# carlosmwh1985/BspAtom

Hardware: AMD Instinct MI355X
Metric: l-channel eigensolves/sec at N_bsp=4096 fp64 (higher is better)
Workload: dtype f64; 1 GPU; Hydrogen Coulomb l=0..127, N_bsp=4096, k=9, KIND_GRID=0 rb=800 (BASELINE configs[3]); `value` = weak scaling: 128 l-channels per GPU, 128 in total; channels_total=128, eigenvector_owner_rank=0, collective_calls=0, launched_by=python

## Files before the change

bspatom_amd/csrc/capi.hip:

```cpp
#include <atomic>
#include <new>
#include "capi_internal.h"

using namespace bsp;

namespace bsp {
static std::atomic<int> g_process_device{-1};
int process_device() { return g_process_device.load(); }
int process_device_check(int device)
{
    const int cur = g_process_device.load();
    if (cur >= 0 && cur != device) {
        fprintf(stderr, "bspatom: this process already works on device %d; use one process per GPU (device %d refused)\n", cur, device);
        return BSP_ERR_UNSUPPORTED;
    }
    return BSP_OK;
}
void process_device_latch(int device) { int expect = -1; g_process_device.compare_exchange_strong(expect, device); }
}

namespace {
struct OptName { const char *name; const char *env; int Options::*field; };
const OptName OPT_TABLE[] = {
    {"sb2st_version", "BSP_SB2ST_VERSION", &Options::sb2st_version},
    {"sb2st_ring", "BSP_SB2ST_RING", &Options::sb2st_ring},
    {"sb2st_margin", "BSP_SB2ST_MARGIN", &Options::sb2st_margin},
    {"sb2st_hyst", "BSP_SB2ST_HYST", &Options::sb2st_hyst},
    {"sb2st_lead", "BSP_SB2ST_LEAD", &Options::sb2st_lead},
    {"sb2st_check", "BSP_SB2ST_CHECK", &Options::sb2st_check},
    {"sb2st_diag", "BSP_SB2ST_DIAG", &Options::sb2st_diag},
    {"sb2st_force_abort", "BSP_SB2ST_FORCE_ABORT", &Options::sb2st_force_abort},
    {"sy2sb_groups", "BSP_SY2SB_GROUPS", &Options::sy2sb_groups},
    {"sy2sb_lookahead", "BSP_SY2SB_LOOKAHEAD", &Options::sy2sb_lookahead},
    {"sy2sb_segs", "BSP_SY2SB_SEGS", &Options::sy2sb_segs},
    {"panel_qr", "BSP_PANEL_QR", &Options::panel_qr},
    {"gemm_diag", "BSP_GEMM_DIAG", &Options::gemm_diag},
    {"bisect", "BSP_BISECT", &Options::bisect},
    {"bisect_ept", "BSP_BISECT_EPT", &Options::bisect_ept},
    {"bisect_tail", "BSP_BISECT_TAIL", &Options::bisect_tail},
    {"bisect_secant", "BSP_BISECT_SECANT", &Options::bisect_secant},
    {"bisect_pair", "BSP_BISECT_PAIR", &Options::bisect_pair},
    {"bisect_queue", "BSP_BISECT_QUEUE", &Options::bisect_queue},
    {"bisect_queue_grid", "BSP_BISECT_QUEUE_GRID", &Options::bisect_queue_grid},
    {"bisect_diag", "BSP_BISECT_DIAG", &Options::bisect_diag},
    {"no_eigvec_prefetch", "BSP_NO_EIGVEC_PREFETCH", &Options::no_eigvec_prefetch},
    {"vec_early", "BSP_VEC_EARLY", &Options::vec_early},
    {"vec_own_cu", "BSP_VEC_OWN_CU", &Options::vec_own_cu},
    {"poison_c", "BSP_POISON_C", &Options::poison_c},
    {"sb2sb_mfma", "BSP_SB2SB_MFMA", &Options::sb2sb_mfma},
    {"ktime", "BSP_KTIME", &Options::ktime},
    {"tsqr_regcap", "BSP_TSQR_REGCAP", &Options::tsqr_regcap},
    {"tsqr_max_m", "BSP_TSQR_MAX_M", &Options::tsqr_max_m},
    {"sb16_rows", "BSP_SB16_ROWS", &Options::sb16_rows},
    {"route", "BSP_ROUTE", &Options::route},
    {"cw_onediv", "BSP_CW_ONEDIV", &Options::cw_onediv},
    {"cw_items4", "BSP_CW_ITEMS4", &Options::cw_items4},
    {"cw_nw", "BSP_CW_NW", &Options::cw_nw},
    {"cw_ldspad", "BSP_CW_LDSPAD", &Options::cw_ldspad},
    {"cw_ipw", "BSP_CW_IPW", &Options::cw_ipw},
    {"cw_band8", "BSP_CW_BAND8", &Options::cw_band8},
    {"cw_split", "BSP_CW_SPLIT", &Options::cw_split},
    {"cw_diag", "BSP_CW_DIAG", &Options::cw_diag},
    {"s_overlap", "BSP_S_OVERLAP", &Options::s_overlap},
    {"cw_streams", "BSP_CW_STREAMS", &Options::cw_streams},
    {"cw_chunk_min", "BSP_CW_CHUNK_MIN", &Options::cw_chunk_min},
    {"sb8_wgs", "BSP_SB8_WGS", &Options::sb8_wgs},
    {"sbr_phased", "BSP_SBR_PHASED", &Options::sbr_phased},
    {"sbr_lag", "BSP_SBR_LAG", &Options::sbr_lag},
    {"fused_probe", "BSP_FUSED_PROBE", &Options::fused_probe},
    {"dipole_stage_mb", "BSP_DIPOLE_STAGE_MB", &Options::dipole_stage_mb},
    {"wf_stage_mb", "BSP_WF_STAGE_MB", &Options::wf_stage_mb},
    {"tdse_stage_mb", "BSP_TDSE_STAGE_MB", &Options::tdse_stage_mb},
    {"tdse_adapt_group", "BSP_TDSE_ADAPT_GROUP", &Options::tdse_adapt_group},
};
}

namespace bsp {
Options &opts()
{
    static Options o = [] {
        Options v;
        for (const OptName &t : OPT_TABLE) {
            const char *e = getenv(t.env);
            if (e) v.*(t.field) = (*e == 0) ? 1 : atoi(e);
        }
        return v;
    }();
    return o;
}

namespace {
struct KRec { int slot; hipEvent_t e0, e1; };
std::vector<KRec> g_krecs;
std::vector<hipEvent_t> g_kpool;
hipEvent_t g_kopen[KS_COUNT];
hipEvent_t kevent()
{
    hipEvent_t e = nullptr;
    if (!g_kpool.empty()) { e = g_kpool.back(); g_kpool.pop_back(); }
    else if (hipEventCreate(&e) != hipSuccess) e = nullptr;
    return e;
}
const char *const KSLOT_NAMES[KS_COUNT] = {"gemm2_kernel<128,128,MODE 1> (rank-128 update, syr2k)", "gemm2_kernel<64,128,MODE 2> (symm Y = A22 W)",
                                          "panel_qr2_kernel / panel_qr_kernel", "sy2sb chain: G, K (split-K gemm_kernel + splitk_reduce), form_T, tsmm64 (W, Z)",
                                          "sb2sb_mfma_kernel (band 64 -> 16)", "sbr_rows_kernel<8> / <16> / sb16st_kernel (one-column chase to tridiagonal)", "bisect3_kernel",
                                          "band_cholesky_kernel + std_form_kernel",
                                          "crawford_item_kernel and its set-up kernels (band route: pencil -> band 15)",
                                          "operator_band_kernel (bands of caller-given g(r), g(r) d/dr)",
                                          "tdse_stage_kernel (one Runge-Kutta stage of bspatom_tdse_propagate)"};
}
void ktime_begin(int slot, hipStream_t st)
{
    hipEvent_t e = kevent();
    g_kopen[slot] = e;
    if (e) (void)hipEventRecord(e, st);
}
void ktime_end(int slot, hipStream_t st)
{
    hipEvent_t e0 = g_kopen[slot], e1 = kevent();
    g_kopen[slot] = nullptr;
    if (!e0 || !e1) return;
    (void)hipEventRecord(e1, st);
    g_krecs.push_back({slot, e0, e1});
}
}

extern "C" int bspatom_kernel_times(double *ms, int32_t *launches, int cap)
{
    if (!ms || !launches || cap < KS_COUNT) return BSP_ERR_ARG;
    BSP_HIP(hipDeviceSynchronize());
    for (int i = 0; i < cap; ++i) { ms[i] = 0.0; launches[i] = 0; }
    for (const auto &r : g_krecs) {
        float t = 0.f;
        if (hipEventElapsedTime(&t, r.e0, r.e1) == hipSuccess) { ms[r.slot] += t; launches[r.slot] += 1; }
        g_kpool.push_back(r.e0); g_kpool.push_back(r.e1);
    }
    g_krecs.clear();
    return KS_COUNT;
}
// ... 469 lines not shown
```

bspatom_amd/csrc/common.h:

```cpp
#pragma once
#include <hip/hip_runtime.h>
#include <cstdint>
#include <cstdio>
#include <cstdlib>

#define BSP_OK 0
#define BSP_ERR_HIP (-1)
#define BSP_ERR_ARG (-2)
#define BSP_ERR_BSPLVB (-3)
#define BSP_ERR_NOGPU (-4)
#define BSP_ERR_UNSUPPORTED (-5)

#define BSP_HIP(x)                                                                          \
    do {                                                                                    \
        hipError_t e_ = (x);                                                                \
        if (e_ != hipSuccess) {                                                             \
            fprintf(stderr, "bspatom: HIP error '%s' at %s:%d\n", hipGetErrorString(e_),    \
                    __FILE__, __LINE__);                                                    \
            return BSP_ERR_HIP;                                                             \
        }                                                                                   \
    } while (0)

typedef double double4_t __attribute__((ext_vector_type(4)));

__host__ __device__ inline size_t ab_stride(int npad) { return (size_t)npad * 128 + 1088; }

namespace bsp {

struct Options {
    int sb2st_version = 0;
    int sb2st_ring = 0;
    int sb2st_margin = 3, sb2st_hyst = 2;
    int sb2st_lead = 0;
    int sb2st_check = 0;
    int sb2st_diag = 0;
    int sb2st_force_abort = 0;
    int sy2sb_groups = 2, sy2sb_lookahead = 1, sy2sb_segs = 0;
    int panel_qr = 3;
    int tsqr_max_m = 2048;
    int tsqr_regcap = 1;
    int gemm_diag = 0;
    int bisect = 3, bisect_ept = 0;
    int bisect_secant = 1;
    int bisect_tail = 1;
    int bisect_pair = 1;
    int bisect_queue = 1;
    int bisect_queue_grid = 0;
    int bisect_diag = 0;
    int no_eigvec_prefetch = 0;
    int vec_early = 1;
    int vec_own_cu = 1;
    int sb2sb_mfma = 1;
    int sb16_rows = 1;
    int poison_c = 0;
    int route = 0;
    int fused_probe = 0;
    int cw_items4 = 1;
    int cw_nw = 1;
    int cw_streams = 2;
    int cw_chunk_min = 1024;
    int s_overlap = 1;
    int cw_diag = 0;
    int cw_split = 0;
    int cw_band8 = 1;
    int sb8_wgs = 0;
    int sbr_phased = 1;
    int sbr_lag = 0;
    int cw_ipw = 0;
    int cw_ldspad = 0;
    int cw_onediv = 0;
    int dipole_stage_mb = 0;
    int wf_stage_mb = 0;
    int tdse_stage_mb = 0;
    int tdse_adapt_group = 0;
    int ktime = 0;
};
Options &opts();

int process_device();
int process_device_check(int device);
void process_device_latch(int device);

enum KSlot { KS_SYR2K = 0, KS_SYMM, KS_PANEL_QR, KS_CHAIN, KS_SB2SB, KS_SB16ST, KS_BISECT, KS_STDFORM, KS_CRAWFORD, KS_OPBAND, KS_TDSE, KS_COUNT };
void ktime_begin(int slot, hipStream_t st);
void ktime_end(int slot, hipStream_t st);
struct KScope {
    int slot; hipStream_t st; bool on;
    KScope(int slot_, hipStream_t st_) : slot(slot_), st(st_), on(opts().ktime != 0) { if (on) ktime_begin(slot, st); }
    ~KScope() { if (on) ktime_end(slot, st); }
};

struct GemmDesc {
    int M, N, K, batch;
    const double *A; long sAm, sAk, bA;
    const double *B; long sBk, sBn, bB;
    double *C; long sCm, sCn, bC;
    double alpha, beta;
    int lower_only;
    int yoff;
    int ksplit;
    int kchunk;
    long bCs;
    int nsb, toff;
    int sbpre[80];
    int sbxy[80];
};
int gemm_f64(const GemmDesc &g, hipStream_t st);
int gemm_splitk_f64(const GemmDesc &g, int splits, double *part, hipStream_t st);
int tsmm64_f64(int m, int batch, const double *A, long lda, long bsA, const double *B, long bsB, double *C, long ldc, long bsC,
               double alpha, double beta, hipStream_t st);
int syr2k_lower_f64(int m, int batch, double *A22, long ld, long bsA, const double *buf, long ldb, long bsBuf, int seg, int nseg,
                    int part, hipStream_t st);
int symm_lower_f64(int m, int batch, const double *A22, long ld, long bsA, const double *W, long ldw, long bsW,
                   double *Y, long ldy, long bsY, hipStream_t st);

int launch_point_table(int nkp, int k, int ka, int nfun, const double *d_rt, const double *d_aind,
                       const double *d_xg, const double *d_wg, const double *d_vpot, double *d_ptab,
                       int *d_left, int *d_status, hipStream_t st);
int launch_assemble_bands(int nfun, int k, int ka, int nkp, int kind_pot, const double *d_bl, int l0,
                          int nl, const double *d_ptab, const int *d_left, double *d_SB, double *d_HB,
                          hipStream_t st);
int launch_dipole_bands(int nfun, int k, int ka, int nkp, const double *d_ptab, const int *d_left, double *d_RB,
                        hipStream_t st);
int launch_band_cholesky(int n, int k, const double *d_SB, double *d_UB, double *d_rdiag, int *d_info,
                         hipStream_t st);
int launch_band_cholesky_range(int n, int k, int jstart, int jstop, const double *d_SB, double *d_UB, double *d_rdiag, int *d_info,
                               hipStream_t st);
int launch_band_cholesky_pair(int n, int k, int jstop, const double *d_SB, double *d_UB, double *d_rdiag, int *d_info, hipStream_t st);
int launch_standard_form(int n, int npad, int k, int nl, const double *d_HB, const double *d_UB,
                         const double *d_rdiag, double *d_Y, double *d_C, hipStream_t st, int full = 0);
struct CrawfordWork {
    double *SBf, *UBf, *rdiagf;
    double *Qel, *LiB;
    double *D, *E, *G;
    int *info;
};
bool crawford_supported(int n, int k);
size_t crawford_work_bytes(int n, int k, int nl);
void crawford_carve(void *base, int n, int k, int nl, CrawfordWork *w);
constexpr int CW_CHUNKS = 4;
int crawford_prepare(int n, int k, const double *d_SB, const CrawfordWork &w, hipStream_t st, hipEvent_t *evc = nullptr);
int crawford_run(int n, int npad, int k, int nl, const double *d_SB, const double *d_HB, const CrawfordWork &w, double *d_AB,
                 hipStream_t st, bool s_prepared = false, hipEvent_t *evc = nullptr, hipStream_t aux0 = nullptr);
long tsqr_scr_doubles(int npad);
long tsqr_cntr_ints(int npad);
int tsqr_panel(int npad, int r0, int c0, int batch, double *d_A, double *buf, double *W, double *scr, int *cntr, hipStream_t st);
struct Sy2sbWork {
    double *tsqr_scr;
    int *tsqr_cntr;
    double *buf2;
    double *tau2;
    double *buf;
    double *W;
// ... 124 lines not shown
```

bspatom_amd/csrc/crawford.hip:

```cpp
#include "common.h"
#include <cstdio>
#include <mutex>

namespace bsp {
namespace {

constexpr int CB = 8;
constexpr int CBB = CB * CB;

template <int CTRL>
__device__ __forceinline__ double cw_dpp(double x)
{
    union { double d; int i[2]; } u, r;
    u.d = x;
    r.i[0] = __builtin_amdgcn_update_dpp(0, u.i[0], CTRL, 0xf, 0xf, true);
    r.i[1] = __builtin_amdgcn_update_dpp(0, u.i[1], CTRL, 0xf, 0xf, true);
    return r.d;
}
__device__ __forceinline__ double cw_rowsum(double x)
{
    x += cw_dpp<0x128>(x);
    x += cw_dpp<0x124>(x);
    x += cw_dpp<0x122>(x);
    x += cw_dpp<0x121>(x);
// ... 146 lines not shown
        for (int r = 0; r < 2; ++r) {
            if (!elim) Em[(4 * r + g) * CB + c8] = O[r];
            Gm[(4 * r + g) * CB + c8] = O[r + 2];
        }
    }
    if (!elim) {
        if (!left) {
            double *E1 = E + (size_t)(p + 1) * CBB;
            E1[g * CB + c8] = x0;
            E1[(4 + g) * CB + c8] = x1;
        }
    } else if (has_x) {
        double4_t T = {0.0, 0.0, 0.0, 0.0};
        T = cw_mfma(q[2], xt[0], T);
        T = cw_mfma(q[3], xt[1], T);
        if (left) {
            double *Ej = E + (size_t)j * CBB;
#pragma unroll
            for (int r = 0; r < 2; ++r) Ej[c8 * CB + 4 * r + g] = T[r + 2];
        }
    }
}

constexpr int QLD = 18;

template <int I, bool ONEDIV>
__device__ __forceinline__ void rq4_step(double (&x)[16], double (&q)[16], double *bc, const int r)
{
    constexpr int LEN = CB + I;
    if (r == I) {
#pragma unroll
        for (int c = 0; c < 16; c += 2) *reinterpret_cast<double2 *>(bc + c) = make_double2(x[c], x[c + 1]);
    }
    asm volatile("" ::: "memory");
    double u[16];
#pragma unroll
    for (int c = 0; c < 16; c += 2) {
        if (c <= LEN) {
            const double2 v = *reinterpret_cast<const double2 *>(bc + c);
            u[c] = v.x; u[c + 1] = v.y;
        }
    }
    asm volatile("" ::: "memory");
    double sg[4] = {0.0, 0.0, 0.0, 0.0};
#pragma unroll
    for (int c = 0; c < LEN; ++c) sg[c & 3] = fma(u[c], u[c], sg[c & 3]);
    const double sig = (sg[0] + sg[1]) + (sg[2] + sg[3]);
    const double alpha = u[LEN];
    const double a2s = fma(alpha, alpha, sig);
    const bool ok = (a2s > 1e-280) && (sig != 0.0);
    const double nrm = sqrt(ok ? a2s : 1.0);
    const double bt = (alpha >= 0.0) ? -nrm : nrm;
    const double amb = alpha - bt;
    const double okf = ok ? 1.0 : 0.0, ambs = ok ? amb : 1.0, bts = ok ? bt : 1.0;
    const double sc = ONEDIV ? 1.0 : (1.0 / ambs) * okf;
    const double t = (ONEDIV ? -1.0 / (bts * ambs) : (bts - alpha) / bts) * okf;
    const double beta = ok ? bt : alpha;
    if (!ONEDIV) {
#pragma unroll
        for (int c = 0; c < LEN; ++c) u[c] *= sc;
    }
    u[LEN] = ONEDIV ? amb : 1.0;
    {
        double ws[4] = {0.0, 0.0, 0.0, 0.0};
#pragma unroll
        for (int c = 0; c <= LEN; ++c) ws[c & 3] = fma(x[c], u[c], ws[c & 3]);
        const double w = (ws[0] + ws[1]) + (ws[2] + ws[3]);
        const double tw = (r <= I) ? -t * w : 0.0;
#pragma unroll
        for (int c = 0; c <= LEN; ++c) x[c] = fma(tw, u[c], x[c]);
    }
    (void)beta;
    {
        double ws[4] = {0.0, 0.0, 0.0, 0.0};
#pragma unroll
        for (int c = 0; c <= LEN; ++c) ws[c & 3] = fma(q[c], u[c], ws[c & 3]);
        const double w = (ws[0] + ws[1]) + (ws[2] + ws[3]);
        const double tw = -t * w;
#pragma unroll
        for (int c = 0; c <= LEN; ++c) q[c] = fma(tw, u[c], q[c]);
    }
}

template <bool ONEDIV>
__device__ __forceinline__ void cw_quad(const int N, const int t, const int jlo, int nch, int jel, const int ipw, const int nlh,
                                        const int qstride, const int nlead, const int chan, const int idx0, const int lane,
                                        double *Qsw, double *Bcw, double *Wsw, const double *__restrict__ Qel, double *Dall, double *Eall,
                                        double *Gall, unsigned long long *diag)
{
    unsigned long long ts0 = 0, tsa = 0, tsb = 0, tsc = 0, tsd = 0, tse = 0;
    if (diag) ts0 = __builtin_amdgcn_s_memtime();
    if (chan >= nlh) {
        if (jlo + nch > nlead) nch = nlead > jlo ? nlead - jlo : 0;
        if (jel >= nlead) jel = 0;
    }
    const int items = nch + (jel > 0 ? 1 : 0);
    if (idx0 >= items) return;
    const size_t chn = (size_t)chan * N * CBB;
    double *D = Dall + chn, *E = Eall + chn, *G = Gall + chn;

#pragma unroll
    for (int s = 0; s < 4; ++s) {
        const int idx = idx0 + s;
        const int kd = s >= ipw ? 0 : (idx < nch ? 1 : ((idx == nch && jel > 0) ? 2 : 0));
        if (kd != 0) {
            const int jx = kd == 1 ? jlo + idx : jel, p = kd == 2 ? jel - 1 : jx - 2 - (t - 2 * jx);
            const double *srcD = D + (size_t)p * CBB + 2 * lane;
            const double *srcE = E + (size_t)((lane < 32 || p < 1) ? p : p - 1) * CBB + 2 * (lane & 31);
            const unsigned ldsD = (unsigned)(size_t)(__attribute__((address_space(3))) void *)(Wsw + s * 4 * CBB);
            asm volatile("s_mov_b32 m0, %2\n\ts_nop 0\n\tglobal_load_lds_dwordx4 %0, off\n\t"
                         "s_mov_b32 m0, %3\n\ts_nop 0\n\tglobal_load_lds_dwordx4 %1, off"
                         :: "v"(srcD), "v"(srcE), "s"(ldsD), "s"(ldsD + 2 * CBB * 8) : "memory", "m0");
        }
    }

    if (idx0 < nch) {
        const int it = lane >> 4, r = lane & 15;
        const int idx = idx0 + it;
        const bool live = idx < nch && it < ipw && r < CB;
        const int j = jlo + (idx < nch ? idx : 0), p = j - 2 - (t - 2 * j);
        double x[16], q[16];
        {
            const double *gp = G + (size_t)p * CBB + (r & 7) * CB, *ep = E + (size_t)(p + 1) * CBB + (r & 7) * CB;
#pragma unroll
            for (int c = 0; c < CB; c += 2) {
                const double2 a = *reinterpret_cast<const double2 *>(gp + c), b = *reinterpret_cast<const double2 *>(ep + c);
                x[c] = live ? a.x : 0.0; x[c + 1] = live ? a.y : 0.0;
                x[CB + c] = live ? b.x : 0.0; x[CB + c + 1] = live ? b.y : 0.0;
            }
        }
#pragma unroll
        for (int c = 0; c < 16; ++c) q[c] = (c == r) ? 1.0 : 0.0;
        double *bc = Bcw + it * 16;
        if (diag) { asm volatile("s_waitcnt vmcnt(0)" ::: "memory"); tsa = __builtin_amdgcn_s_memtime(); }
        rq4_step<7, ONEDIV>(x, q, bc, r);
        rq4_step<6, ONEDIV>(x, q, bc, r);
        rq4_step<5, ONEDIV>(x, q, bc, r);
        rq4_step<4, ONEDIV>(x, q, bc, r);
        rq4_step<3, ONEDIV>(x, q, bc, r);
        rq4_step<2, ONEDIV>(x, q, bc, r);
        rq4_step<1, ONEDIV>(x, q, bc, r);
        rq4_step<0, ONEDIV>(x, q, bc, r);
        if (diag) { asm volatile("s_waitcnt lgkmcnt(0)" ::: "memory"); tsb = __builtin_amdgcn_s_memtime(); }
        if (live) {
            double *ep = E + (size_t)(p + 1) * CBB + r * CB;
#pragma unroll
            for (int c = 0; c < CB; c += 2) *reinterpret_cast<double2 *>(ep + c) = make_double2(x[CB + c], x[CB + c + 1]);
        }
        double *qs = Qsw + it * (16 * QLD) + r * QLD;
#pragma unroll
        for (int c = 0; c < 16; c += 2) *reinterpret_cast<double2 *>(qs + c) = make_double2(q[c], q[c + 1]);
    }
    if (idx0 < nch) asm volatile("s_waitcnt vmcnt(4) lgkmcnt(0)" ::: "memory");
    else asm volatile("s_waitcnt vmcnt(0) lgkmcnt(0)" ::: "memory");
    if (diag) tsc = __builtin_amdgcn_s_memtime();
    int idx0b = idx0;
    size_t chnb = chn;
    asm volatile("" : "+s"(idx0b), "+s"(chnb));
    D = Dall + chnb; E = Eall + chnb; G = Gall + chnb;

    const int g = lane >> 4, c = lane & 15, c8 = c & 7;
    const bool left = c < CB;
    int kind[4], jj[4], pp[4];
    double wv[4][4], sdv[4][2], qe[4], xt[2] = {0.0, 0.0};
#pragma unroll
    for (int s = 0; s < 4; ++s) {
        const int idx = idx0b + s;
        kind[s] = s >= ipw ? 0 : (idx < nch ? 1 : ((idx == nch && jel > 0) ? 2 : 0));
        jj[s] = kind[s] == 1 ? jlo + idx : (kind[s] == 2 ? jel : jlo + idx0b);
        pp[s] = kind[s] == 2 ? jel - 1 : jj[s] - 2 - (t - 2 * jj[s]);
        if (kind[s] == 0) { jj[s] = jj[0]; pp[s] = pp[0]; }
        const int p = pp[s];
        const double *W0 = Wsw + s * 4 * CBB, *W1 = W0 + CBB, *WE = W0 + 2 * CBB, *WM = W0 + 3 * CBB;
#pragma unroll
        for (int r = 0; r < 2; ++r) {
            const int R = 4 * r + g;
            const int hi = R > c8 ? R : c8, lo = R > c8 ? c8 : R;
            wv[s][r] = *(left ? W0 + hi * CB + lo : WE + c8 * CB + R);
            wv[s][r + 2] = *(left ? WE + R * CB + c8 : W1 + hi * CB + lo);
            const double v = WM[(4 * r + g) * CB + c8];
            sdv[s][r] = (p >= 1 && left) ? v : 0.0;
        }
    }
    int se = -1;
#pragma unroll
    for (int s = 0; s < 4; ++s) if (kind[s] == 2) se = s;
    const bool has_x = se >= 0 && (jel + 1 <= N - 1);
    if (se >= 0) {
        const double *Qj = Qel + ((int)chan >= nlh ? qstride : 0) + (size_t)jel * 256;
#pragma unroll
        for (int r = 0; r < 4; ++r) qe[r] = Qj[(4 * r + g) * 16 + c];
        const double *Ej = E + (size_t)(has_x ? jel : 0) * CBB;
#pragma unroll
        for (int r = 0; r < 2; ++r) {
            const double v = Ej[c8 * CB + 4 * r + g];
            xt[r] = (has_x && left) ? v : 0.0;
        }
    }
    if (diag) { asm volatile("s_waitcnt vmcnt(0)" ::: "memory"); tsd = __builtin_amdgcn_s_memtime(); }
#pragma unroll
    for (int s = 0; s < 4; ++s) {
        if (kind[s] == 0) break;
        const bool elim = kind[s] == 2;
        const int p = pp[s];
        double *D0 = D + (size_t)p * CBB, *D1 = D0 + CBB, *E0 = E + (size_t)p * CBB;
        double q[4];
        if (!elim) {
            const double *qs = Qsw + s * (16 * QLD);
#pragma unroll
            for (int r = 0; r < 4; ++r) q[r] = qs[(4 * r + g) * QLD + c];
        } else {
#pragma unroll
            for (int r = 0; r < 4; ++r) q[r] = qe[r];
        }
        double4_t P = {0.0, 0.0, 0.0, 0.0}, Wn = {0.0, 0.0, 0.0, 0.0};
#pragma unroll
        for (int r = 0; r < 4; ++r) P = cw_mfma(wv[s][r], q[r], P);
#pragma unroll
        for (int r = 0; r < 4; ++r) Wn = cw_mfma(q[r], P[r], Wn);
        double4_t O = {0.0, 0.0, 0.0, 0.0};
        O = cw_mfma(q[0], sdv[s][0], O);
        O = cw_mfma(q[1], sdv[s][1], O);
        if (left) {
#pragma unroll
            for (int r = 0; r < 2; ++r) {
                D0[(4 * r + g) * CB + c8] = Wn[r];
                E0[(4 * r + g) * CB + c8] = Wn[r + 2];
            }
        } else {
#pragma unroll
            for (int r = 0; r < 2; ++r) D1[(4 * r + g) * CB + c8] = Wn[r + 2];
        }
        if (p >= 1 && left) {
            double *Em = E + (size_t)(p - 1) * CBB, *Gm = G + (size_t)(p - 1) * CBB;
#pragma unroll
            for (int r = 0; r < 2; ++r) {
                if (!elim) Em[(4 * r + g) * CB + c8] = O[r];
                Gm[(4 * r + g) * CB + c8] = O[r + 2];
            }
        }
        if (elim && has_x) {
            double4_t T = {0.0, 0.0, 0.0, 0.0};
            T = cw_mfma(q[2], xt[0], T);
            T = cw_mfma(q[3], xt[1], T);
            if (left) {
                double *Ej = E + (size_t)jel * CBB;
#pragma unroll
                for (int r = 0; r < 2; ++r) Ej[c8 * CB + 4 * r + g] = T[r + 2];
            }
        }
    }
    if (diag) {
        tse = __builtin_amdgcn_s_memtime();
        asm volatile("s_waitcnt vmcnt(0)" ::: "memory");
        const unsigned long long tsf = __builtin_amdgcn_s_memtime();
        if (lane == 0) {
            const bool a = tsa != 0;
            atomicAdd(diag + 0, a ? tsa - ts0 : 0ull);
            atomicAdd(diag + 1, a ? tsb - tsa : 0ull);
            atomicAdd(diag + 2, a ? tsc - tsb : tsc - ts0);
            atomicAdd(diag + 3, tsd - tsc);
            atomicAdd(diag + 4, tse - tsd);
            atomicAdd(diag + 5, tsf - tse);
            atomicAdd(diag + 6, tsf - ts0);
            atomicAdd(diag + 7, 1ull);
        }
    }
}

template <bool ONEDIV, int NW>
__global__ __launch_bounds__(64 * NW, 8 / NW) void crawford_item4_kernel(int N, int t, int jlo, int nch, int jel, int ipw, int nlh, int qstride,
                                                            int nlead, const double *__restrict__ Qel, double *Dall, double *Eall, double *Gall,
                                                            unsigned long long *diag)
{
    __builtin_amdgcn_s_setprio(3);
    if (diag && (((blockIdx.x & 7) | (blockIdx.y & 7)) != 0)) diag = nullptr;
    __shared__ __attribute__((aligned(16))) double Qs[NW][4][16 * QLD];
    __shared__ __attribute__((aligned(16))) double Bc[NW][4][16];
    __shared__ __attribute__((aligned(16))) double Ws[NW][4][4 * CBB];
    const int lane = threadIdx.x & 63;
    const int wave = __builtin_amdgcn_readfirstlane(threadIdx.x >> 6);
    cw_quad<ONEDIV>(N, t, jlo, nch, jel, ipw, nlh, qstride, nlead, (int)blockIdx.y, (blockIdx.x * NW + wave) * ipw, lane, &Qs[wave][0][0],
                    &Bc[wave][0][0], &Ws[wave][0][0], Qel, Dall, Eall, Gall, diag);
}

__global__ void crawford_flip_kernel(int n, int k, const double *__restrict__ SB, double *__restrict__ SBf)
{
    const int idx = blockIdx.x * blockDim.x + threadIdx.x;
    if (idx >= n * k) return;
    const int d = idx / n, i = idx % n;
    SBf[idx] = (i + d < n) ? SB[(size_t)d * n + (n - 1 - i - d)] : 0.0;
    SBf[(size_t)n * k + idx] = SB[idx];
}

__global__ __launch_bounds__(64) void crawford_setup_kernel(int n, int k, int fstride, int jfirst, const double *__restrict__ UB0,
                                                           double *__restrict__ LiB0, double *__restrict__ Qel0)
{
    __shared__ double Ld[CB][CB + 1], M[CB][CB + 1], Li[CB][CB + 1];
    const int j = jfirst + blockIdx.x, t = threadIdx.x, r = t >> 3, c = t & 7, b = k - 1;
    const double *UBf = UB0 + (size_t)blockIdx.y * k * n;
    double *LiB = LiB0 + (size_t)blockIdx.y * fstride * CBB, *Qel = Qel0 + (size_t)blockIdx.y * fstride * 256;
    const int i = CB * j + r;
    {
        const int ic = CB * j + c, d = r - c;
        double v = 0.0;
        if (i >= n) v = (r == c) ? 1.0 : 0.0;
        else if (d >= 0 && d <= b) v = UBf[(size_t)d * n + ic];
        Ld[r][c] = v;
        const int im = CB * (j - 1) + c, dm = CB + r - c;
        double m = 0.0;
        if (j > 0 && i < n && dm <= b) m = UBf[(size_t)dm * n + im];
        M[r][c] = m;
        Li[r][c] = 0.0;
    }
    __syncthreads();
    if (t < CB) {
        double x[CB];
#pragma unroll
        for (int rr = 0; rr < CB; ++rr) {
            double s = (rr == t) ? 1.0 : 0.0;
#pragma unroll
            for (int kk = 0; kk < CB; ++kk)
                if (kk < rr && kk >= t) s -= Ld[rr][kk] * x[kk];
            x[rr] = (rr >= t) ? s / Ld[rr][rr] : 0.0;
        }
#pragma unroll
        for (int rr = 0; rr < CB; ++rr) Li[rr][t] = x[rr];
    }
    __syncthreads();
    double kv = 0.0;
#pragma unroll
    for (int kk = 0; kk < CB; ++kk) kv += Li[r][kk] * M[kk][c];
    LiB[(size_t)j * CBB + t] = Li[r][c];
    double *Q = Qel + (size_t)j * 256;
    Q[r * 16 + c] = (r == c) ? 1.0 : 0.0;
    Q[c * 16 + CB + r] = -kv;
    Q[(CB + r) * 16 + c] = 0.0;
    Q[(CB + c) * 16 + CB + r] = Li[r][c];
}

__global__ __launch_bounds__(64) void crawford_init_kernel(int n, int k, int N, int nlh, int listride, const double *__restrict__ HBall,
                                                          const double *__restrict__ LiB, double *Dall, double *Eall)
{
    __shared__ double Ds[CB][CB + 1], Es[CB][CB + 1], Ls[CB][CB + 1], Ts[CB][CB + 1];
    const int p = blockIdx.x, t = threadIdx.x, r = t >> 3, c = t & 7, b = k - 1;
    const bool fwd = (int)blockIdx.y >= nlh;
    const double *HB = HBall + (size_t)(fwd ? blockIdx.y - nlh : blockIdx.y) * k * n;
    auto Hf = [&](int i, int i2) -> double {
        const int hi = i > i2 ? i : i2, lo = i > i2 ? i2 : i, d = hi - lo;
        return (hi < n && d <= b) ? HB[(size_t)d * n + (fwd ? lo : n - 1 - hi)] : 0.0;
    };
    double dv = Hf(CB * p + r, CB * p + c), ev = Hf(CB * (p + 1) + r, CB * p + c);
    if (p == 0) {
        Ds[r][c] = dv; Es[r][c] = ev; Ls[r][c] = LiB[(fwd ? listride : 0) + t];
        __syncthreads();
        double s = 0.0, e2 = 0.0;
#pragma unroll
        for (int kk = 0; kk < CB; ++kk) { s += Ls[r][kk] * Ds[kk][c]; e2 += Es[r][kk] * Ls[c][kk]; }
        Ts[r][c] = s;
        __syncthreads();
        s = 0.0;
#pragma unroll
        for (int kk = 0; kk < CB; ++kk) s += Ts[r][kk] * Ls[c][kk];
        dv = s; ev = e2;
    }
    const size_t o = ((size_t)blockIdx.y * N + p) * CBB + t;
// ... 199 lines not shown
{
    CwShape c;
    c.N = (n + CB - 1) / CB;
    c.Nl = (opts().cw_split > 0 && n % CB == 0) ? (int)((long)c.N * (opts().cw_split > 50 ? 50 : opts().cw_split) / 100) : 0;
    c.split = c.Nl >= 3 && c.N - c.Nl >= 4;
    if (!c.split) c.Nl = 0;
    c.Nh = c.split ? c.N - c.Nl : 0;
    c.Nproc = c.split ? c.Nh : c.N;
    c.Ns = c.split ? c.Nh + 2 : c.N;
    return c;
}
int cw_chunk_cols(int n) { return n < opts().cw_chunk_min ? n + 128 : ((n + CW_CHUNKS - 1) / CW_CHUNKS + 127) / 128 * 128; }
}

int crawford_prepare(int n, int k, const double *d_SB, const CrawfordWork &w, hipStream_t st, hipEvent_t *evc)
{
    if (!crawford_supported(n, k)) return BSP_ERR_UNSUPPORTED;
    const CwShape c = cw_shape(n);
    const int N = c.N, Nh = c.Nh, Nl = c.Nl;
    int rc;
    BSP_HIP(hipMemsetAsync(w.info, 0, sizeof(int), st));
    hipLaunchKernelGGL(crawford_flip_kernel, dim3((n * k + 255) / 256), dim3(256), 0, st, n, k, d_SB, w.SBf);
    if (c.split) {
        if ((rc = launch_band_cholesky_pair(n, k, CB * Nh, w.SBf, w.UBf, w.rdiagf, w.info, st))) return rc;
        hipLaunchKernelGGL(crawford_setup_kernel, dim3(Nh, 2), dim3(64), 0, st, n, k, N, 0, w.UBf, w.LiB, w.Qel);
        hipLaunchKernelGGL(crawford_cut_setup_kernel, dim3(1), dim3(64), 0, st, n, k, N, Nh, Nl, w.SBf, w.LiB, w.Qel, w.info);
    } else if (evc) {
        const int cc = cw_chunk_cols(n);
        for (int q = 0, j0 = 0; q < CW_CHUNKS; ++q, j0 += cc) {
            if (j0 < n) {
                const int j1 = j0 + cc < n ? j0 + cc : n, b0 = j0 / CB, b1 = j1 < n ? j1 / CB : N;
                if ((rc = launch_band_cholesky_range(n, k, j0, j1, w.SBf, w.UBf, w.rdiagf, w.info, st))) return rc;
                hipLaunchKernelGGL(crawford_setup_kernel, dim3(b1 - b0, 1), dim3(64), 0, st, n, k, N, b0, w.UBf, w.LiB, w.Qel);
            }
            BSP_HIP(hipEventRecord(evc[q], st));
        }
    } else {
        if ((rc = launch_band_cholesky(n, k, w.SBf, w.UBf, w.rdiagf, w.info, st))) return rc;
        hipLaunchKernelGGL(crawford_setup_kernel, dim3(N, 1), dim3(64), 0, st, n, k, N, 0, w.UBf, w.LiB, w.Qel);
    }
    if (evc && c.split)
        for (int q = 0; q < CW_CHUNKS; ++q) BSP_HIP(hipEventRecord(evc[q], st));
    BSP_HIP(hipGetLastError());
    return BSP_OK;
}

int crawford_run(int n, int npad, int k, int nl, const double *d_SB, const double *d_HB, const CrawfordWork &w, double *d_AB,
                 hipStream_t st, bool s_prepared, hipEvent_t *evc, hipStream_t aux0)
{
    if (!crawford_supported(n, k)) return BSP_ERR_UNSUPPORTED;
    const int N = (n + CB - 1) / CB;
    int Nl = (opts().cw_split > 0 && n % CB == 0) ? (int)((long)N * (opts().cw_split > 50 ? 50 : opts().cw_split) / 100) : 0;
    const bool split = Nl >= 3 && N - Nl >= 4;
    if (!split) Nl = 0;
    const int Nh = split ? N - Nl : 0;
    const int Nproc = split ? Nh : N;
    const int Ns = split ? Nh + 2 : N;
    const int ny = split ? 2 * nl : nl;
    const int nlead = split ? Nl : 0x7fffffff;
    int rc;
    KScope kt(KS_CRAWFORD, st);
    if (!s_prepared && (rc = crawford_prepare(n, k, d_SB, w, st))) return rc;
    if (!s_prepared) evc = nullptr;
    const int ccb = cw_chunk_cols(n) / CB;
    int waited = 0;
    if (evc) BSP_HIP(hipStreamWaitEvent(st, evc[0], 0));
    hipLaunchKernelGGL(crawford_init_kernel, dim3(Nproc, ny), dim3(64), 0, st, n, k, Ns, nl, N * CBB, d_HB, w.LiB, w.D, w.E);
    BSP_HIP(hipGetLastError());
    const int qstride = N * 256;
    unsigned long long *dg = nullptr;
    if (opts().cw_diag && opts().cw_items4) {
        BSP_HIP(hipMalloc(reinterpret_cast<void **>(&dg), 8 * sizeof(unsigned long long)));
        BSP_HIP(hipMemsetAsync(dg, 0, 8 * sizeof(unsigned long long), st));
    }
    auto wavefront = [&](int t, int jlo, int nch, int jel, int cy, int c0 = 0, hipStream_t ws = nullptr) {
        if (!ws) ws = st;
        double *gD = w.D + (size_t)c0 * Ns * CBB, *gE = w.E + (size_t)c0 * Ns * CBB, *gG = w.G + (size_t)c0 * Ns * CBB;
        const int items = nch + (jel ? 1 : 0);
        if (opts().cw_items4) {
            const int nw = opts().cw_nw == 4 ? 4 : 1;
            const int ipw = (opts().cw_ipw == 1 || opts().cw_ipw == 2) ? opts().cw_ipw : 4;
            const int waves = (items + ipw - 1) / ipw;
            const dim3 grid((waves + nw - 1) / nw, cy), block(64 * nw);
            if (opts().cw_onediv) hipLaunchKernelGGL((crawford_item4_kernel<true, 1>), dim3(waves, cy), dim3(64), 0, ws, Ns, t, jlo, nch, jel, ipw, nl, qstride, nlead, w.Qel, gD, gE, gG, dg);
            else if (nw == 4) hipLaunchKernelGGL((crawford_item4_kernel<false, 4>), grid, block, 0, ws, Ns, t, jlo, nch, jel, ipw, nl, qstride, nlead, w.Qel, gD, gE, gG, dg);
            else hipLaunchKernelGGL((crawford_item4_kernel<false, 1>), grid, block, (size_t)opts().cw_ldspad * 1024, ws, Ns, t, jlo, nch, jel, ipw, nl, qstride, nlead, w.Qel, gD, gE, gG, dg);
        } else {
            const dim3 grid((items + 3) / 4, cy);
            if (opts().cw_onediv) hipLaunchKernelGGL(crawford_item_kernel<true>, grid, dim3(256), 0, ws, Ns, t, jlo, nch, jel, nl, qstride, nlead, w.Qel, gD, gE, gG);
            else hipLaunchKernelGGL(crawford_item_kernel<false>, grid, dim3(256), 0, ws, Ns, t, jlo, nch, jel, nl, qstride, nlead, w.Qel, gD, gE, gG);
        }
    };
    const int tmax = (Nproc >= 3) ? 3 * Nproc - 5 : (Nproc == 2 ? 1 : 0);
    int ngrp = 1;
    if (!split && !dg && opts().cw_streams > 1) {
        ngrp = opts().cw_streams > 4 ? 4 : opts().cw_streams;
        while (ngrp > 1 && nl / ngrp < 16) --ngrp;
    }
    static hipStream_t s_aux[3] = {nullptr, nullptr, nullptr};
    hipStream_t aux[3];
    hipEvent_t evf = nullptr, evj[3] = {nullptr, nullptr, nullptr};
    if (ngrp > 1) {
        static std::mutex mx;
        std::lock_guard<std::mutex> lk(mx);
        for (int g = 0; g < ngrp - 1; ++g)
            if (!s_aux[g] && !(g == 0 && aux0)) BSP_HIP(hipStreamCreateWithFlags(&s_aux[g], hipStreamNonBlocking));
        for (int g = 0; g < 3; ++g) aux[g] = (g == 0 && aux0) ? aux0 : s_aux[g];
        BSP_HIP(hipEventCreateWithFlags(&evf, hipEventDisableTiming));
        BSP_HIP(hipEventRecord(evf, st));
        for (int g = 0; g < ngrp - 1; ++g) BSP_HIP(hipStreamWaitEvent(aux[g], evf, 0));
    }
    for (int t = 1; t <= tmax; ++t) {
        const int jel = ((t & 1) && (t + 1) / 2 <= Nproc - 1) ? (t + 1) / 2 : 0;
        const int jlo = (t + 2 + 2) / 3;
        const int jhi = (t / 2 < Nproc - 1) ? t / 2 : Nproc - 1;
        const int nch = (jhi >= jlo && jlo >= 2) ? jhi - jlo + 1 : 0;
        if (nch + (jel ? 1 : 0) == 0) continue;
        if (evc && jel) {
            const int q = jel / ccb < CW_CHUNKS - 1 ? jel / ccb : CW_CHUNKS - 1;
            for (; waited < q; ++waited)
                for (int g = 0; g < ngrp; ++g) BSP_HIP(hipStreamWaitEvent(g == 0 ? st : aux[g - 1], evc[waited + 1], 0));
        }
        for (int g = 0; g < ngrp; ++g) {
            const int c0 = (int)((long)ny * g / ngrp), c1 = (int)((long)ny * (g + 1) / ngrp);
            wavefront(t, jlo, nch, jel, c1 - c0, c0, g == 0 ? st : aux[g - 1]);
        }
    }
    if (ngrp > 1) {
        for (int g = 0; g < ngrp - 1; ++g) {
            BSP_HIP(hipEventCreateWithFlags(&evj[g], hipEventDisableTiming));
            BSP_HIP(hipEventRecord(evj[g], aux[g]));
            BSP_HIP(hipStreamWaitEvent(st, evj[g], 0));
        }
        hipEventDestroy(evf);
        for (int g = 0; g < ngrp - 1; ++g) hipEventDestroy(evj[g]);
    }
    if (evc)
        for (; waited < CW_CHUNKS - 1; ++waited) BSP_HIP(hipStreamWaitEvent(st, evc[waited + 1], 0));
    if (split) {
        hipLaunchKernelGGL(crawford_cut_prep_kernel, dim3(nl), dim3(64), 0, st, Ns, Nh, Nl, nl, N, w.LiB, w.D, w.E);
        wavefront(2 * Nh - 1, 0, 0, Nh, nl);
        for (int sft = 0; sft <= Nh - 2; ++sft) wavefront(2 * Nh + sft, Nh, 1, 0, nl);
    }
    BSP_HIP(hipGetLastError());
    if (dg) {
        unsigned long long h[8];
        BSP_HIP(hipStreamSynchronize(st));
        BSP_HIP(hipMemcpy(h, dg, sizeof(h), hipMemcpyDeviceToHost));
        hipFree(dg);
        const double wv = h[7] ? (double)h[7] : 1.0;
        fprintf(stderr, "crawford_item4_kernel, %llu waves, s_memtime ticks per wave: X arrives %.0f | eight reflectors %.0f | R, Q stored %.0f | "
                        "phase B operands arrive %.0f | congruences issued %.0f | stores leave %.0f | wave %.0f\n", h[7], h[0] / wv, h[1] / wv,
                h[2] / wv, h[3] / wv, h[4] / wv, h[5] / wv, h[6] / wv);
    }
    const bool band8 = opts().cw_band8 != 0;
    if (band8) hipLaunchKernelGGL(crawford_corner_kernel, dim3(ny), dim3(64), 0, st, Ns, w.D, w.E);
    hipLaunchKernelGGL(crawford_band_kernel, dim3((npad * 32 + 255) / 256, nl), dim3(256), 0, st, n, npad, Ns, band8 ? CB : 2 * CB - 1,
                       Nh, N, nl, w.D, w.E, d_AB);
    BSP_HIP(hipGetLastError());
    return BSP_OK;
}

}
```

Measured before the change: 2064 eigensolves/s.

## Broadcast Householder pivots via DPP row_newbcast instead of LDS in Crawford quad

Adds a BCAST variant of the Crawford item kernel that broadcasts the Householder sigma/alpha and reflector components within each 16-lane row using v_fmac_f64_dpp and v_mov_b64_dpp with row_newbcast, in place of a round trip through LDS. It also hoists the phase-B operand reads earlier, right after the E store, so they overlap outstanding memory ops. Phase B reuses the Q LDS slot, which shrinks the kernel's LDS footprint, and launch bounds raise the occupancy hint from 8 to 16 waves. The variant is on by default; it depends on hand-written inline asm with s_nop hazard padding and on correct waitcnt ordering.

```diff
diff --git a/bspatom_amd/csrc/capi.hip b/bspatom_amd/csrc/capi.hip
--- a/bspatom_amd/csrc/capi.hip
+++ b/bspatom_amd/csrc/capi.hip
@@ -55,6 +55,7 @@
     {"route", "BSP_ROUTE", &Options::route},
     {"cw_onediv", "BSP_CW_ONEDIV", &Options::cw_onediv},
     {"cw_items4", "BSP_CW_ITEMS4", &Options::cw_items4},
+    {"cw_bcast", "BSP_CW_BCAST", &Options::cw_bcast},
     {"cw_nw", "BSP_CW_NW", &Options::cw_nw},
     {"cw_ldspad", "BSP_CW_LDSPAD", &Options::cw_ldspad},
     {"cw_ipw", "BSP_CW_IPW", &Options::cw_ipw},
diff --git a/bspatom_amd/csrc/common.h b/bspatom_amd/csrc/common.h
--- a/bspatom_amd/csrc/common.h
+++ b/bspatom_amd/csrc/common.h
@@ -69,6 +69,7 @@
     int cw_ipw = 0;
     int cw_ldspad = 0;
     int cw_onediv = 0;
+    int cw_bcast = 1;
     int dipole_stage_mb = 0;
     int wf_stage_mb = 0;
     int tdse_stage_mb = 0;
diff --git a/bspatom_amd/csrc/crawford.hip b/bspatom_amd/csrc/crawford.hip
--- a/bspatom_amd/csrc/crawford.hip
+++ b/bspatom_amd/csrc/crawford.hip
@@ -252,7 +252,117 @@
     }
 }
 
-template <bool ONEDIV>
+#define CW_PAD "s_nop 1\n\t"
+#define CW_DPPC " row_newbcast:%[I] row_mask:0xf bank_mask:0xf\n\t"
+#define CW_FD(a, k) "v_fmac_f64_dpp %[a" #a "], %[u" #k "], %[x" #k "]" CW_DPPC
+#define CW_FA(k) "v_fmac_f64_dpp %[x" #k "], %[u" #k "], %[tw]" CW_DPPC
+#define CW_FD1 CW_FD(0, 0)
+#define CW_FD2 CW_FD1 CW_FD(1, 1)
+#define CW_FD3 CW_FD2 CW_FD(2, 2)
+#define CW_FD4 CW_FD3 CW_FD(3, 3)
+#define CW_FD5 CW_FD4 CW_FD(0, 4)
+#define CW_FD6 CW_FD5 CW_FD(1, 5)
+#define CW_FD7 CW_FD6 CW_FD(2, 6)
+#define CW_FD8 CW_FD7 CW_FD(3, 7)
+#define CW_FA1 CW_FA(0)
+#define CW_FA2 CW_FA1 CW_FA(1)
+#define CW_FA3 CW_FA2 CW_FA(2)
+#define CW_FA4 CW_FA3 CW_FA(3)
+#define CW_FA5 CW_FA4 CW_FA(4)
+#define CW_FA6 CW_FA5 CW_FA(5)
+#define CW_FA7 CW_FA6 CW_FA(6)
+#define CW_FA8 CW_FA7 CW_FA(7)
+#define CW_UI(k) [u##k] "v"(u[O + k])
+#define CW_XI(k) [x##k] "v"(x[O + k])
+#define CW_XO(k) [x##k] "+v"(x[O + k])
+#define CW_L1(M) M(0)
+#define CW_L2(M) CW_L1(M), M(1)
+#define CW_L3(M) CW_L2(M), M(2)
+#define CW_L4(M) CW_L3(M), M(3)
+#define CW_L5(M) CW_L4(M), M(4)
+#define CW_L6(M) CW_L5(M), M(5)
+#define CW_L7(M) CW_L6(M), M(6)
+#define CW_L8(M) CW_L7(M), M(7)
+#define CW_DOT_CASE(n)                                                                                                               \
+    if constexpr (CNT == n)                                                                                                          \
+        asm(CW_PAD CW_FD##n : [a0] "+v"(ws[0]), [a1] "+v"(ws[1]), [a2] "+v"(ws[2]), [a3] "+v"(ws[3])                           \
+            : CW_L##n(CW_UI), CW_L##n(CW_XI), [I] "i"(I));
+#define CW_AXPY_CASE(n)                                                                                                              \
+    if constexpr (CNT == n) asm(CW_PAD CW_FA##n : CW_L##n(CW_XO) : CW_L##n(CW_UI), [tw] "v"(tw), [I] "i"(I));
+#define CW_AXPYL_CASE(n)                                                                                                             \
+    if constexpr (CNT == n)                                                                                                          \
+        asm(CW_PAD CW_FA##n "v_fmac_f64 %[xl], %[nt], %[w]\n\t" : CW_L##n(CW_XO), [xl] "+v"(x[O + n])                                  \
+            : CW_L##n(CW_UI), [tw] "v"(tw), [nt] "v"(nt), [w] "v"(w), [I] "i"(I));
+
+template <int I, int O, int CNT>
+__device__ __forceinline__ void cw_bdot(double (&ws)[4], const double (&u)[16], const double (&x)[16])
+{
+    static_assert(CNT >= 1 && CNT <= 8 && (O & 3) == 0, "a statement of at most eight FMAs");
+    CW_DOT_CASE(1) CW_DOT_CASE(2) CW_DOT_CASE(3) CW_DOT_CASE(4) CW_DOT_CASE(5) CW_DOT_CASE(6) CW_DOT_CASE(7) CW_DOT_CASE(8)
+}
+template <int I, int O, int CNT>
+__device__ __forceinline__ void cw_baxpy(double (&x)[16], const double (&u)[16], const double tw)
+{
+    static_assert(CNT >= 1 && CNT <= 8, "a statement of at most eight FMAs");
+    CW_AXPY_CASE(1) CW_AXPY_CASE(2) CW_AXPY_CASE(3) CW_AXPY_CASE(4) CW_AXPY_CASE(5) CW_AXPY_CASE(6) CW_AXPY_CASE(7) CW_AXPY_CASE(8)
+}
+
+template <int I, int O, int CNT>
+__device__ __forceinline__ void cw_baxpy_last(double (&x)[16], const double (&u)[16], const double tw, const double nt, const double w)
+{
+    static_assert(CNT >= 1 && CNT <= 7, "a statement of at most eight FMAs");
+    CW_AXPYL_CASE(1) CW_AXPYL_CASE(2) CW_AXPYL_CASE(3) CW_AXPYL_CASE(4) CW_AXPYL_CASE(5) CW_AXPYL_CASE(6) CW_AXPYL_CASE(7)
+}
+
+template <int I, bool ONEDIV>
+__device__ __forceinline__ void rq4_step_dpp(double (&x)[16], double (&q)[16], const int r)
+{
+    constexpr int LEN = CB + I;
+    double sg[4] = {0.0, 0.0, 0.0, 0.0};
+#pragma unroll
+    for (int c = 0; c < LEN; ++c) sg[c & 3] = fma(x[c], x[c], sg[c & 3]);
+    const double sigl = (sg[0] + sg[1]) + (sg[2] + sg[3]), alphal = x[LEN];
+    double sig, alpha;
+    asm(CW_PAD
+        "v_mov_b64_dpp %[s], %[sl]" CW_DPPC "v_mov_b64_dpp %[a], %[al]" CW_DPPC
+        : [s] "=&v"(sig), [a] "=&v"(alpha) : [sl] "v"(sigl), [al] "v"(alphal), [I] "i"(I));
+    const double a2s = fma(alpha, alpha, sig);
+    const bool ok = (a2s > 1e-280) && (sig != 0.0);
+    const double nrm = sqrt(ok ? a2s : 1.0);
+    const double bt = (alpha >= 0.0) ? -nrm : nrm;
+    const double amb = alpha - bt;
+    const double okf = ok ? 1.0 : 0.0, ambs = ok ? amb : 1.0, bts = ok ? bt : 1.0;
+    const double sc = ONEDIV ? 1.0 : (1.0 / ambs) * okf;
+    const double t = (ONEDIV ? -1.0 / (bts * ambs) : (bts - alpha) / bts) * okf;
+    double u[16];
+#pragma unroll
+    for (int c = 0; c < 16; ++c) u[c] = (c < LEN) ? (ONEDIV ? x[c] : x[c] * sc) : (ONEDIV ? amb : 1.0);
+    {
+        double ws[4] = {0.0, 0.0, 0.0, 0.0};
+        cw_bdot<I, 0, 8>(ws, u, x);
+        cw_bdot<I, 8, I + 1>(ws, u, x);
+        const double w = (ws[0] + ws[1]) + (ws[2] + ws[3]);
+        const double tw = (r <= I) ? -t * w : 0.0;
+        cw_baxpy<I, 0, 8>(x, u, tw);
+        cw_baxpy<I, 8, I + 1>(x, u, tw);
+    }
+    {
+        double ws[4] = {0.0, 0.0, 0.0, 0.0};
+        cw_bdot<I, 0, 8>(ws, u, q);
+        cw_bdot<I, 8, I + 1>(ws, u, q);
+        const double w = (ws[0] + ws[1]) + (ws[2] + ws[3]);
+        const double tw = -t * w;
+        cw_baxpy<I, 0, 8>(q, u, tw);
+        if constexpr (ONEDIV) {
+            cw_baxpy<I, 8, I + 1>(q, u, tw);
+        } else {
+            if constexpr (I > 0) cw_baxpy_last<I, 8, I>(q, u, tw, -t, w);
+            else q[LEN] = fma(-t, w, q[LEN]);
+        }
+    }
+}
+
+template <bool ONEDIV, bool BCAST>
 __device__ __forceinline__ void cw_quad(const int N, const int t, const int jlo, int nch, int jel, const int ipw, const int nlh,
                                         const int qstride, const int nlead, const int chan, const int idx0, const int lane,
                                         double *Qsw, double *Bcw, double *Wsw, const double *__restrict__ Qel, double *Dall, double *Eall,
@@ -284,6 +394,24 @@
         }
     }
 
+    double wv[4][4], sdv[4][2];
+    auto read_ws = [&]() {
+        const int g = lane >> 4, c8 = lane & 7;
+        const bool left = (lane & 15) < CB;
+#pragma unroll
+        for (int s = 0; s < 4; ++s) {
+            const double *W0 = Wsw + s * 4 * CBB, *W1 = W0 + CBB, *WE = W0 + 2 * CBB, *WM = W0 + 3 * CBB;
+#pragma unroll
+            for (int r = 0; r < 2; ++r) {
+                const int R = 4 * r + g;
+                const int hi = R > c8 ? R : c8, lo = R > c8 ? c8 : R;
+                wv[s][r] = *(left ? W0 + hi * CB + lo : WE + c8 * CB + R);
+                wv[s][r + 2] = *(left ? WE + R * CB + c8 : W1 + hi * CB + lo);
+                sdv[s][r] = WM[(4 * r + g) * CB + c8];
+            }
+        }
+    };
+
     if (idx0 < nch) {
         const int it = lane >> 4, r = lane & 15;
         const int idx = idx0 + it;
@@ -301,27 +429,47 @@
         }
 #pragma unroll
         for (int c = 0; c < 16; ++c) q[c] = (c == r) ? 1.0 : 0.0;
-        double *bc = Bcw + it * 16;
         if (diag) { asm volatile("s_waitcnt vmcnt(0)" ::: "memory"); tsa = __builtin_amdgcn_s_memtime(); }
-        rq4_step<7, ONEDIV>(x, q, bc, r);
-        rq4_step<6, ONEDIV>(x, q, bc, r);
-        rq4_step<5, ONEDIV>(x, q, bc, r);
-        rq4_step<4, ONEDIV>(x, q, bc, r);
-        rq4_step<3, ONEDIV>(x, q, bc, r);
-        rq4_step<2, ONEDIV>(x, q, bc, r);
-        rq4_step<1, ONEDIV>(x, q, bc, r);
-        rq4_step<0, ONEDIV>(x, q, bc, r);
+        if constexpr (BCAST) {
+            rq4_step_dpp<7, ONEDIV>(x, q, r);
+            rq4_step_dpp<6, ONEDIV>(x, q, r);
+            rq4_step_dpp<5, ONEDIV>(x, q, r);
+            rq4_step_dpp<4, ONEDIV>(x, q, r);
+            rq4_step_dpp<3, ONEDIV>(x, q, r);
+            rq4_step_dpp<2, ONEDIV>(x, q, r);
+            rq4_step_dpp<1, ONEDIV>(x, q, r);
+            rq4_step_dpp<0, ONEDIV>(x, q, r);
+        } else {
+            double *bc = Bcw + it * 16;
+            rq4_step<7, ONEDIV>(x, q, bc, r);
+            rq4_step<6, ONEDIV>(x, q, bc, r);
+            rq4_step<5, ONEDIV>(x, q, bc, r);
+            rq4_step<4, ONEDIV>(x, q, bc, r);
+            rq4_step<3, ONEDIV>(x, q, bc, r);
+            rq4_step<2, ONEDIV>(x, q, bc, r);
+            rq4_step<1, ONEDIV>(x, q, bc, r);
+            rq4_step<0, ONEDIV>(x, q, bc, r);
+        }
         if (diag) { asm volatile("s_waitcnt lgkmcnt(0)" ::: "memory"); tsb = __builtin_amdgcn_s_memtime(); }
         if (live) {
             double *ep = E + (size_t)(p + 1) * CBB + r * CB;
 #pragma unroll
             for (int c = 0; c < CB; c += 2) *reinterpret_cast<double2 *>(ep + c) = make_double2(x[CB + c], x[CB + c + 1]);
         }
+        if constexpr (BCAST) {
+            asm volatile("s_waitcnt vmcnt(4)" ::: "memory");
+            read_ws();
+            asm volatile("" ::: "memory");
+        }
         double *qs = Qsw + it * (16 * QLD) + r * QLD;
 #pragma unroll
         for (int c = 0; c < 16; c += 2) *reinterpret_cast<double2 *>(qs + c) = make_double2(q[c], q[c + 1]);
-    }
-    if (idx0 < nch) asm volatile("s_waitcnt vmcnt(4) lgkmcnt(0)" ::: "memory");
+    } else if constexpr (BCAST) {
+        asm volatile("s_waitcnt vmcnt(0)" ::: "memory");
+        read_ws();
+    }
+    if constexpr (BCAST) asm volatile("s_waitcnt lgkmcnt(0)" ::: "memory");
+    else if (idx0 < nch) asm volatile("s_waitcnt vmcnt(4) lgkmcnt(0)" ::: "memory");
     else asm volatile("s_waitcnt vmcnt(0) lgkmcnt(0)" ::: "memory");
     if (diag) tsc = __builtin_amdgcn_s_memtime();
     int idx0b = idx0;
@@ -332,7 +480,8 @@
     const int g = lane >> 4, c = lane & 15, c8 = c & 7;
     const bool left = c < CB;
     int kind[4], jj[4], pp[4];
-    double wv[4][4], sdv[4][2], qe[4], xt[2] = {0.0, 0.0};
+    double qe[4], xt[2] = {0.0, 0.0};
+    if constexpr (!BCAST) read_ws();
 #pragma unroll
     for (int s = 0; s < 4; ++s) {
         const int idx = idx0b + s;
@@ -340,17 +489,8 @@
         jj[s] = kind[s] == 1 ? jlo + idx : (kind[s] == 2 ? jel : jlo + idx0b);
         pp[s] = kind[s] == 2 ? jel - 1 : jj[s] - 2 - (t - 2 * jj[s]);
         if (kind[s] == 0) { jj[s] = jj[0]; pp[s] = pp[0]; }
-        const int p = pp[s];
-        const double *W0 = Wsw + s * 4 * CBB, *W1 = W0 + CBB, *WE = W0 + 2 * CBB, *WM = W0 + 3 * CBB;
-#pragma unroll
-        for (int r = 0; r < 2; ++r) {
-            const int R = 4 * r + g;
-            const int hi = R > c8 ? R : c8, lo = R > c8 ? c8 : R;
-            wv[s][r] = *(left ? W0 + hi * CB + lo : WE + c8 * CB + R);
-            wv[s][r + 2] = *(left ? WE + R * CB + c8 : W1 + hi * CB + lo);
-            const double v = WM[(4 * r + g) * CB + c8];
-            sdv[s][r] = (p >= 1 && left) ? v : 0.0;
-        }
+#pragma unroll
+        for (int r = 0; r < 2; ++r) sdv[s][r] = (pp[s] >= 1 && left) ? sdv[s][r] : 0.0;
     }
     int se = -1;
 #pragma unroll
@@ -438,20 +578,23 @@
     }
 }
 
-template <bool ONEDIV, int NW>
-__global__ __launch_bounds__(64 * NW, 8 / NW) void crawford_item4_kernel(int N, int t, int jlo, int nch, int jel, int ipw, int nlh, int qstride,
+template <bool ONEDIV, int NW, bool BCAST>
+__global__ __launch_bounds__(64 * NW, (BCAST ? 16 : 8) / NW) void crawford_item4_kernel(int N, int t, int jlo, int nch, int jel, int ipw, int nlh, int qstride,
                                                             int nlead, const double *__restrict__ Qel, double *Dall, double *Eall, double *Gall,
                                                             unsigned long long *diag)
 {
     __builtin_amdgcn_s_setprio(3);
     if (diag && (((blockIdx.x & 7) | (blockIdx.y & 7)) != 0)) diag = nullptr;
     __shared__ __attribute__((aligned(16))) double Qs[NW][4][16 * QLD];
-    __shared__ __attribute__((aligned(16))) double Bc[NW][4][16];
-    __shared__ __attribute__((aligned(16))) double Ws[NW][4][4 * CBB];
+    __shared__ __attribute__((aligned(16))) double Bc[BCAST ? 1 : NW][BCAST ? 1 : 4][BCAST ? 2 : 16];
+    __shared__ __attribute__((aligned(16))) double Wsep[BCAST ? 1 : NW][BCAST ? 1 : 4][BCAST ? 2 : 4 * CBB];
+    static_assert(16 * QLD >= 4 * CBB, "a slot of Q holds a slot of phase B's operands");
+    double *Wsw = BCAST ? &Qs[0][0][0] : &Wsep[0][0][0];
     const int lane = threadIdx.x & 63;
     const int wave = __builtin_amdgcn_readfirstlane(threadIdx.x >> 6);
-    cw_quad<ONEDIV>(N, t, jlo, nch, jel, ipw, nlh, qstride, nlead, (int)blockIdx.y, (blockIdx.x * NW + wave) * ipw, lane, &Qs[wave][0][0],
-                    &Bc[wave][0][0], &Ws[wave][0][0], Qel, Dall, Eall, Gall, diag);
+    cw_quad<ONEDIV, BCAST>(N, t, jlo, nch, jel, ipw, nlh, qstride, nlead, (int)blockIdx.y, (blockIdx.x * NW + wave) * ipw, lane,
+                           &Qs[wave][0][0], BCAST ? nullptr : &Bc[wave][0][0], Wsw + wave * (BCAST ? 4 * 16 * QLD : 4 * 4 * CBB), Qel, Dall,
+                           Eall, Gall, diag);
 }
 
 __global__ void crawford_flip_kernel(int n, int k, const double *__restrict__ SB, double *__restrict__ SBf)
@@ -817,9 +960,19 @@
             const int ipw = (opts().cw_ipw == 1 || opts().cw_ipw == 2) ? opts().cw_ipw : 4;
             const int waves = (items + ipw - 1) / ipw;
             const dim3 grid((waves + nw - 1) / nw, cy), block(64 * nw);
-            if (opts().cw_onediv) hipLaunchKernelGGL((crawford_item4_kernel<true, 1>), dim3(waves, cy), dim3(64), 0, ws, Ns, t, jlo, nch, jel, ipw, nl, qstride, nlead, w.Qel, gD, gE, gG, dg);
-            else if (nw == 4) hipLaunchKernelGGL((crawford_item4_kernel<false, 4>), grid, block, 0, ws, Ns, t, jlo, nch, jel, ipw, nl, qstride, nlead, w.Qel, gD, gE, gG, dg);
-            else hipLaunchKernelGGL((crawford_item4_kernel<false, 1>), grid, block, (size_t)opts().cw_ldspad * 1024, ws, Ns, t, jlo, nch, jel, ipw, nl, qstride, nlead, w.Qel, gD, gE, gG, dg);
+            const size_t pad = (size_t)opts().cw_ldspad * 1024;
+#define CW_LAUNCH4(OD, NWV, BC, G, B, LDS)                                                                                           \
+    hipLaunchKernelGGL((crawford_item4_kernel<OD, NWV, BC>), G, B, LDS, ws, Ns, t, jlo, nch, jel, ipw, nl, qstride, nlead, w.Qel, gD, gE, gG, dg)
+            if (opts().cw_bcast) {
+                if (opts().cw_onediv) CW_LAUNCH4(true, 1, true, dim3(waves, cy), dim3(64), 0);
+                else if (nw == 4) CW_LAUNCH4(false, 4, true, grid, block, 0);
+                else CW_LAUNCH4(false, 1, true, grid, block, pad);
+            } else {
+                if (opts().cw_onediv) CW_LAUNCH4(true, 1, false, dim3(waves, cy), dim3(64), 0);
+                else if (nw == 4) CW_LAUNCH4(false, 4, false, grid, block, 0);
+                else CW_LAUNCH4(false, 1, false, grid, block, pad);
+            }
+#undef CW_LAUNCH4
         } else {
             const dim3 grid((items + 3) / 4, cy);
             if (opts().cw_onediv) hipLaunchKernelGGL(crawford_item_kernel<true>, grid, dim3(256), 0, ws, Ns, t, jlo, nch, jel, nl, qstride, nlead, w.Qel, gD, gE, gG);
```

Result: faster. 2111 eigensolves/s, median of 6 (+2.3%).
